# RIKEN-RCCS/EigenExa

Measured on AMD Instinct MI355X. Metric: eigen_sx full-solve throughput (reference flop model: 4/3 N^3 + D&C GEMM + 2 nvec N^2), higher is better.
Workload: dtype f64; 1 GPU; N=8192 random symmetric fp64 (counter-based R+R^T, seed 20240807), eigen_sx all eigenpairs, m_forward=64, m_backward=128; parallelism=1 GPU (1x1 grid)

## Files before the change

### eigenexa_amd/csrc/api.hip

```cpp
#include "eigx_context.h"
#include "eigx_comm.h"
#include "../../include/eigenexa_amd.h"
#include <cstring>

namespace eigx {
Context g_ctx;
}

using namespace eigx;

extern "C" {

int eigx_init(int device) {
  return eigx_init_multi(device, 0, 1, nullptr, 'C');
}

int eigx_get_device_count(void) {
  int ndev = 0;
  if (hipGetDeviceCount(&ndev) != hipSuccess) { (void)hipGetLastError(); return 0; }
  return ndev;
}

int eigx_get_rccl_unique_id(void* out128) {
  return comm_get_unique_id(out128);
}

static int g_next_px = 0, g_next_py = 0;
int eigx_set_grid_dims(int px, int py) {
  if (px < 0 || py < 0 || (px == 0) != (py == 0)) return EIGX_ERR_BAD_ARG;
  g_next_px = px; g_next_py = py;
  return EIGX_OK;
}

int eigx_init_multi(int device, int rank, int nranks, const void* uid, char order) {
  if (g_ctx.initialized) {
    fprintf(stderr, "[eigx] caution: eigx_init called twice; freeing the previous grid\n");
    eigx_free();
  }
  if (nranks < 1 || rank < 0 || rank >= nranks) return EIGX_ERR_BAD_ARG;
  int ndev = 0;
  if (hipGetDeviceCount(&ndev) != hipSuccess || ndev <= 0) {
    fprintf(stderr, "[eigx] no HIP device visible: this library has no CPU path\n");
    return EIGX_ERR_NO_DEVICE;
  }
  if (device < 0 || device >= ndev) return EIGX_ERR_BAD_ARG;
  EIGX_HIP_CHECK(hipSetDevice(device));
  g_ctx.device = device;
  int Px = 1;
  for (int x = 1; x * x <= nranks; ++x)
    if (nranks % x == 0) Px = x;
  int req_px = 0, req_py = 0;
  if (g_next_px > 0) {
    const int rx = g_next_px, ry = g_next_py;
    req_px = rx; req_py = ry;
    g_next_px = g_next_py = 0;
    if (rx * ry != nranks) {
      fprintf(stderr, "[eigx] illegal grid dimensions %d x %d for %d ranks\n", rx, ry, nranks);
      return EIGX_ERR_BAD_ARG;
    }
    Px = rx;
  }
  Grid g;
  g.Px = Px;
  g.Py = nranks / Px;
  g.rank = rank;
  g.nranks = nranks;
  if (order == 'R' || order == 'r') {
    g.px = rank / g.Py;
    g.py = rank % g.Py;
    g.row_major = 1;
  } else {
    g.px = rank % g.Px;
    g.py = rank / g.Px;
    g.row_major = 0;
  }
  g_ctx.grid = g;
  if (nranks > 1) {
    const int rc = comm_init(g_ctx, uid);
    if (rc != 0) {
      g_ctx.grid = Grid();
      g_next_px = req_px; g_next_py = req_py;
      return rc;
    }
  }
  EIGX_HIP_CHECK(hipStreamCreateWithFlags(&g_ctx.stream, hipStreamNonBlocking));
  EIGX_HIP_CHECK(hipStreamCreateWithFlags(&g_ctx.side_stream, hipStreamNonBlocking));
  for (int q = 0; q < Context::kAux; ++q)
    EIGX_HIP_CHECK(hipStreamCreateWithFlags(&g_ctx.aux[q], hipStreamNonBlocking));
  for (int q = 0; q <= Context::kAux; ++q)
    EIGX_HIP_CHECK(hipEventCreateWithFlags(&g_ctx.aux_ev[q], hipEventDisableTiming));
  EIGX_HIP_CHECK(hipEventCreateWithFlags(&g_ctx.bt_ev, hipEventDisableTiming));
  EIGX_HIP_CHECK(hipEventCreateWithFlags(&g_ctx.dc_ev, hipEventDisableTiming));
  {
    int prio_lo = 0, prio_hi = 0;
    EIGX_HIP_CHECK(hipDeviceGetStreamPriorityRange(&prio_lo, &prio_hi));
    EIGX_HIP_CHECK(hipStreamCreateWithPriority(&g_ctx.dc_stream, hipStreamNonBlocking, prio_hi));
  }
  EIGX_HIP_CHECK(hipEventCreateWithFlags(&g_ctx.dc_b_ev, hipEventDisableTiming));
  EIGX_HIP_CHECK(hipEventCreateWithFlags(&g_ctx.dc_z_ev, hipEventDisableTiming));
  g_ctx.bt_stream = g_ctx.side_stream;
  g_ctx.initialized = true;
  g_ctx.errinfo = 0;
  return EIGX_OK;
}

int eigx_free(void) {
  if (!g_ctx.initialized) return EIGX_OK;
  EIGX_HIP_CHECK(hipSetDevice(g_ctx.device));
  EIGX_HIP_CHECK(hipDeviceSynchronize());
  if (g_ctx.grid.nranks > 1) comm_free(g_ctx);
  g_ctx.pool.release();
  for (hipEvent_t e : g_ctx.prof_ev) EIGX_HIP_CHECK(hipEventDestroy(e));
  EIGX_HIP_CHECK(hipStreamDestroy(g_ctx.stream));
  EIGX_HIP_CHECK(hipStreamDestroy(g_ctx.side_stream));
  for (int q = 0; q < Context::kAux; ++q) EIGX_HIP_CHECK(hipStreamDestroy(g_ctx.aux[q]));
  for (int q = 0; q <= Context::kAux; ++q) EIGX_HIP_CHECK(hipEventDestroy(g_ctx.aux_ev[q]));
  EIGX_HIP_CHECK(hipEventDestroy(g_ctx.bt_ev));
  EIGX_HIP_CHECK(hipEventDestroy(g_ctx.dc_ev));
  EIGX_HIP_CHECK(hipStreamDestroy(g_ctx.dc_stream));
  g_ctx.bt_stream = nullptr;
  EIGX_HIP_CHECK(hipEventDestroy(g_ctx.dc_b_ev));
  EIGX_HIP_CHECK(hipEventDestroy(g_ctx.dc_z_ev));
  g_ctx = Context();
  return EIGX_OK;
}

int eigx_get_version(int* version, char* date32, char* vcode32) {
  if (version) *version = 10;
  if (date32) { memset(date32, 0, 32); strncpy(date32, "2026-10", 31); }
  if (vcode32) { memset(vcode32, 0, 32); strncpy(vcode32, "eigenexa_amd gfx950", 31); }
  return EIGX_OK;
}

int eigx_get_procs(int* procs, int* x_procs, int* y_procs) {
  if (!g_ctx.initialized) return EIGX_ERR_NOT_INITIALIZED;
  if (procs) *procs = g_ctx.grid.nranks;
  if (x_procs) *x_procs = g_ctx.grid.Px;
  if (y_procs) *y_procs = g_ctx.grid.Py;
  return EIGX_OK;
}

int eigx_get_id(int* id, int* x_id, int* y_id) {
  if (!g_ctx.initialized) return EIGX_ERR_NOT_INITIALIZED;
  if (id) *id = g_ctx.grid.rank + 1;
  if (x_id) *x_id = g_ctx.grid.px + 1;
  if (y_id) *y_id = g_ctx.grid.py + 1;
  return EIGX_OK;
}

int eigx_get_comm(int* x_color, int* x_key, int* y_color, int* y_key) {
  if (!g_ctx.initialized) return EIGX_ERR_NOT_INITIALIZED;
  const Grid& g = g_ctx.grid;
  if (x_color) *x_color = g.py + 1;
  if (x_key) *x_key = g.px + 1;
  if (y_color) *y_color = g.px + 1;
  if (y_key) *y_key = g.py + 1;
  return EIGX_OK;
}

double eigx_comm_seconds(void) { return g_ctx.timers[4]; }

int eigx_comm_info(char* buf, int len) {
  if (!g_ctx.initialized) return EIGX_ERR_NOT_INITIALIZED;
  return comm_info(g_ctx, buf, len);
}

int eigx_get_errinfo(int64_t* info) {
  if (info) *info = g_ctx.errinfo;
  return EIGX_OK;
}

int eigx_loop_start(int istart, int nnod, int inod) { return (istart + nnod - 1 - inod) / nnod + 1; }
int eigx_loop_end(int iend, int nnod, int inod) { return (iend + nnod - inod) / nnod; }
int eigx_translate_l2g(int ictr, int nnod, int inod) { return (ictr - 1) * nnod + inod; }
int eigx_translate_g2l(int ictr, int nnod, int inod) { (void)inod; return (ictr - 1) / nnod + 1; }
int eigx_owner_node(int ictr, int nnod, int inod) { (void)inod; return (ictr - 1) % nnod + 1; }
int eigx_owner_index(int ictr, int nnod, int inod) {
  return ((ictr - 1) % nnod + 1 == inod) ? (ictr - 1) / nnod + 1 : -1;
}

int eigx_matdims_for_grid(int n, int x_procs, int y_procs, int m_forward, int m_backward, char mode, int* nx, int* ny) {
  if (!nx || !ny || x_procs < 1 || y_procs < 1) return EIGX_ERR_BAD_ARG;
  (void)m_forward;
  if (n <= 0) { *nx = -1; *ny = -1; return EIGX_ERR_BAD_ARG; }
  const int Px = x_procs, Py = y_procs;
  const int mb = m_backward > 0 ? m_backward : 128;
  const int n1 = ceil_div(n, Px);
  const int n2 = ceil_div(n, Py);
  int lnx;
  int64_t lny;
  if (mode == 'M' || mode == 'm') {
    lnx = n1; lny = n2;
  } else if (mode == 'L' || mode == 'l') {
    lnx = ceil_div(n1, 32) * 32; lny = n2;
  } else {
    lnx = ceil_div(n1, 64) * 64 + 32;
    if (lnx < n1 + 64) lnx += 64;
    const int NB = mb > 64 ? mb : 64;
    int64_t nmz = (int64_t)ceil_div(n1, NB) * NB + 1;
    const int64_t nmz2 = (int64_t)ceil_div(ceil_div(n, NB), Px) * NB;
    if (nmz2 > nmz) nmz = nmz2;
    int64_t nmw = (int64_t)ceil_div(n2, NB) * NB + 1;
    const int64_t nmw2 = (int64_t)ceil_div(ceil_div(n, NB), Py) * NB;
    if (nmw2 > nmw) nmw = nmw2;
    nmz += NB; nmw += NB;
    const int64_t big = nmz > lnx ? nmz : lnx;
    lny = ceil_div64(big * nmw, lnx);
    if (lny < n2) lny = n2;
    lnx = hbm_ld(lnx);
  }
  {
    const int P = Px * Py;
    const int nf = ceil_div(n, P);
    const int64_t nx0 = (int64_t)nf * (P / Px), ny0 = (int64_t)nf * (P / Py);
    if (nx0 > lnx) lnx = (int)nx0;
    if (ny0 > lny) lny = ny0;
  }
  const int pmin = Px < Py ? Px : Py;
  const int64_t side = ceil_div64(ceil_div(n, pmin), 64) * 64;
  if ((side * side >= ((int64_t)1 << 31) || lny >= ((int64_t)1 << 31)) && !(getenv("EIGX_ALLOW_64BIT"))) {
    *nx = -1; *ny = -1;
    return EIGX_ERR_TOO_LARGE;
  }
  *nx = lnx;
  *ny = (int)lny;
  return EIGX_OK;
}

int eigx_get_matdims(int n, int* nx, int* ny, int m_forward, int m_backward, char mode) {
  if (!g_ctx.initialized) return EIGX_ERR_NOT_INITIALIZED;
  return eigx_matdims_for_grid(n, g_ctx.grid.Px, g_ctx.grid.Py, m_forward, m_backward, mode, nx, ny);
}

int64_t eigx_memory_internal(int n, int lda, int ldz, int m_forward, int m_backward) {
  if (!g_ctx.initialized) return -1;
  return solver_workspace_bytes(g_ctx, n, lda, ldz, m_forward, m_backward);
}

int64_t eigx_held_bytes(void) {
  if (!g_ctx.initialized) return -1;
  int64_t t = 0;
  for (const auto& kv : g_ctx.pool.bufs) t += (int64_t)kv.second.bytes;
  return t + comm_held_bytes(g_ctx);
}

int64_t eigx_held_bytes_named(const char* prefix) {
  if (!g_ctx.initialized || !prefix) return -1;
  const std::string pre(prefix);
  int64_t t = 0;
  for (const auto& kv : g_ctx.pool.bufs)
    if (kv.first.compare(0, pre.size(), pre) == 0) t += (int64_t)kv.second.bytes;
  return t;
}

int eigx_get_timers(double* out16) {
  if (!out16) return EIGX_ERR_BAD_ARG;
  for (int i = 0; i < 16; ++i) out16[i] = g_ctx.timers[i];
  return EIGX_OK;
}

int eigx_profile(int stride) {
  if (!g_ctx.initialized) return EIGX_ERR_NOT_INITIALIZED;
  g_ctx.prof_stride = stride > 0 ? stride : 0;
  g_ctx.prof_used = 0;
  g_ctx.prof_kind.clear();
  g_ctx.prof_units.clear();
  return EIGX_OK;
}

int eigx_profile_read(double* out6) {
  if (!g_ctx.initialized) return EIGX_ERR_NOT_INITIALIZED;
  if (!out6) return EIGX_ERR_BAD_ARG;
  EIGX_HIP_CHECK(hipSetDevice(g_ctx.device));
  EIGX_HIP_CHECK(hipStreamSynchronize(g_ctx.stream));
  for (int q = 0; q < 6; ++q) out6[q] = 0.0;
  for (size_t q = 0; q < g_ctx.prof_kind.size(); ++q) {
    float ms = 0.f;
    EIGX_HIP_CHECK(hipEventElapsedTime(&ms, g_ctx.prof_ev[2 * q], g_ctx.prof_ev[2 * q + 1]));
    if (g_ctx.prof_kind[q] > 1) continue;
    const int k = g_ctx.prof_kind[q] ? 3 : 0;
    out6[k + 0] += 1.0;
    out6[k + 1] += g_ctx.prof_units[q];
    out6[k + 2] += 1e-3 * ms;
  }
  return EIGX_OK;
}

int eigx_profile_read_kinds(double* out, int nkinds) {
  if (!g_ctx.initialized) return EIGX_ERR_NOT_INITIALIZED;
  if (!out || nkinds < 1) return EIGX_ERR_BAD_ARG;
  EIGX_HIP_CHECK(hipSetDevice(g_ctx.device));
  EIGX_HIP_CHECK(hipStreamSynchronize(g_ctx.stream));
  for (int q = 0; q < 3 * nkinds; ++q) out[q] = 0.0;
  for (size_t q = 0; q < g_ctx.prof_kind.size(); ++q) {
    const int k = g_ctx.prof_kind[q];
    if (k < 0 || k >= nkinds) continue;
    float ms = 0.f;
    EIGX_HIP_CHECK(hipEventElapsedTime(&ms, g_ctx.prof_ev[2 * q], g_ctx.prof_ev[2 * q + 1]));
    out[3 * k + 0] += 1.0;
    out[3 * k + 1] += g_ctx.prof_units[q];
    out[3 * k + 2] += 1e-3 * ms;
  }
  return EIGX_OK;
}

int eigx_device_synchronize(void) {
  if (!g_ctx.initialized) return EIGX_ERR_NOT_INITIALIZED;
  EIGX_HIP_CHECK(hipSetDevice(g_ctx.device));
  EIGX_HIP_CHECK(hipDeviceSynchronize());
  return EIGX_OK;
}

void* eigx_malloc_dev(int64_t bytes) {
  if (!g_ctx.initialized) return nullptr;
  void* p = nullptr;
  if (hipMalloc(&p, (size_t)bytes) != hipSuccess) return nullptr;
  return p;
}
int eigx_free_dev(void* p) {
  if (p) EIGX_HIP_CHECK(hipFree(p));
  return EIGX_OK;
}
int eigx_memcpy_h2d(void* dst, const void* src, int64_t bytes) {
  EIGX_HIP_CHECK(hipMemcpy(dst, src, (size_t)bytes, hipMemcpyHostToDevice));
  return EIGX_OK;
}
int eigx_memcpy_d2h(void* dst, const void* src, int64_t bytes) {
  EIGX_HIP_CHECK(hipMemcpy(dst, src, (size_t)bytes, hipMemcpyDeviceToHost));
  return EIGX_OK;
}

int eigx_tune(int key, int value) {
  if (key == 0) return set_gemm_variant(value);
  if (key == 1) return set_bisect_threads(value);
  if (key == 2) return set_bt_q(value);
  if (key == 3 || key == 4 || key == 5 || key == 10 || key == 11) return set_reduce_knob(key, value);
  if (key == 12) return (value >= 0 && value <= 2) ? set_reduce_knob(key, value) : -1;
  if (key == 6) return set_gemm_cstream(value);
  if (key == 7) return value > 0 ? set_reduce_knob(key, value) : -1;
  if (key == 8) return set_dc_chunk(value);
  if (key == 9) return comm_set_bounce(value);
  if (key == 15) return set_dc_pipe(value);
  if (key == 16) return set_dc_batch(value);
  if (key == 17 || key == 18 || key == 19) return set_range_knob(key, value);
  if (key == 20) return set_tri_nb(value);
  if (key == 21) return set_batch_nmax(value);
  if (key == 22) return set_hbatch_nmax(value);
  if (key == 23) return set_gbatch_nmax(value);
  if (key == 24) return set_hgbatch_nmax(value);
  return -1;
}

int eigx_dgemm_dev(char opa, char opb, int m, int n, int k, double alpha, const double* a, int lda,
                   const double* b, int ldb, double beta, double* c, int ldc, int tri_upper) {
  if (!g_ctx.initialized) return EIGX_ERR_NOT_INITIALIZED;
  EIGX_HIP_CHECK(hipStreamSynchronize(nullptr));
  dgemm_dev(g_ctx.stream, opa, opb, m, n, k, alpha, a, lda, b, ldb, beta, c, ldc, tri_upper ? 1 : 0,
            &g_ctx.grid);
  EIGX_HIP_CHECK(hipStreamSynchronize(g_ctx.stream));
  return EIGX_OK;
}

int eigx_dgemm_gather_dev(char opa, char opb, int m, int n, int k, double alpha, const double* a, int lda,
                          const double* b, int ldb, double beta, double* c, int ldc, const int* kmap_a,
                          const int* kmap_b) {
  if (!g_ctx.initialized) return EIGX_ERR_NOT_INITIALIZED;
  EIGX_HIP_CHECK(hipStreamSynchronize(nullptr));
  dgemm_dev(g_ctx.stream, opa, opb, m, n, k, alpha, a, lda, b, ldb, beta, c, ldc, 0, nullptr, kmap_a, nullptr, 1, 0,
            0, 0, 1, 0, 0, 0, 1, 0, kmap_b);
  EIGX_HIP_CHECK(hipStreamSynchronize(g_ctx.stream));
  return EIGX_OK;
}

}
```

### eigenexa_amd/csrc/eigx_common.h

```cpp
#pragma once
#include <hip/hip_runtime.h>
#include <cstdio>
#include <cstdlib>
#include <cstdint>
#include <cmath>
#include <vector>
#include <ctime>
#include <chrono>

#define EIGX_HIP_CHECK(expr)                                                        \
  do {                                                                              \
    hipError_t _e = (expr);                                                         \
    if (_e != hipSuccess) {                                                         \
      fprintf(stderr, "[eigx] HIP error %s at %s:%d: %s\n", hipGetErrorName(_e),    \
              __FILE__, __LINE__, hipGetErrorString(_e));                           \
      abort();                                                                      \
    }                                                                               \
  } while (0)

namespace eigx {

typedef double d4_t __attribute__((ext_vector_type(4)));

struct Grid {
  int Px = 1, Py = 1;
  int px = 0, py = 0;
  int rank = 0, nranks = 1;
  int row_major = 0;
};

static inline int ceil_div(int a, int b) { return (a + b - 1) / b; }

static inline int hbm_ld(int l) {
  if (l < 2048) return l;
  const int m = l % 2048;
  if (m < 512) return l + (512 - m);
  if (m > 1536) return l + (2048 - m) + 512;
  return l;
}
static inline int pad_ld(int n) {
  static const int extra = [] { const char* e = getenv("EIGX_LD_EXTRA"); return e ? atoi(e) : 0; }();
  int l = (n + 31) / 32;
  if (l * 32 >= 2048) return hbm_ld(l * 32) + extra;
  if ((l & 1) == 0) ++l;
  return l * 32 + extra;
}
static inline int64_t ceil_div64(int64_t a, int64_t b) { return (a + b - 1) / b; }

static inline int local_count(int n, int P, int p) { return n > p ? (n - p + P - 1) / P : 0; }
static inline int numroc(int n, int nb, int p, int P) {
  const int nblocks = n / nb;
  int cnt = (nblocks / P) * nb;
  const int extra = nblocks % P;
  if (p < extra) cnt += nb;
  else if (p == extra) cnt += n % nb;
  return cnt;
}

inline double now_s() {
  return std::chrono::duration<double>(std::chrono::steady_clock::now().time_since_epoch()).count();
}

struct SolveRequest {
  char mode;
  int nvec;
  bool want_vec;
};
inline char upper_case(char c) { return (c >= 'a' && c <= 'z') ? (char)(c - 'a' + 'A') : c; }
inline SolveRequest normalize_request(int n, int nvec, char mode) {
  mode = upper_case(mode);
  if (nvec == 0) mode = 'N';
  if (nvec < 0) nvec = -nvec;
  if (nvec > n) nvec = n;
  return SolveRequest{mode, nvec, mode != 'N'};
}


__global__ void fill_kernel(double* p, size_t n, double v);
__global__ void fill_vec_kernel(double* __restrict__ w, int n, double v);
__global__ void scale_vec_kernel(double* __restrict__ w, int n, double s);

void dgemm_dev(hipStream_t stream, char opA, char opB, int M, int N, int K, double alpha,
               const double* A, int lda, const double* B, int ldb, double beta, double* C, int ldc,
               int tri_mode = 0, const Grid* g = nullptr, const int* kmapA = nullptr,
               const int* cmapC = nullptr, int batch = 1, long strideA = 0, long strideB = 0, long strideC = 0,
               int batch2 = 1, long strideA2 = 0, long strideB2 = 0, long strideC2 = 0, int ownP = 1,
               int ownp = 0, const int* kmapB = nullptr, int tn_lo = 0, int tn_hi = 0x7fffffff);

struct GemmBatch {
  int M, N, K, pad;
  long offA, offB, offC;
  int offKA, offKB;
};
void dgemm_gather_batch_dev(hipStream_t stream, const GemmBatch* tab_dev, int nbatch, int maxM, int maxN,
                            const double* A, int lda, const double* B, int ldb, double* C, int ldc,
                            const int* kmapA, const int* kmapB);

inline void stage_trace(int rank, const char* what, long detail = -1) {
  static const bool on = getenv("EIGX_TRACE_STAGES") != nullptr;
  if (!on) return;
  timespec ts;
  clock_gettime(CLOCK_MONOTONIC, &ts);
  if (detail >= 0) fprintf(stderr, "[eigx stage] rank %d t=%.3f %s %ld\n", rank, ts.tv_sec % 100000 + ts.tv_nsec * 1e-9, what, detail);
  else fprintf(stderr, "[eigx stage] rank %d t=%.3f %s\n", rank, ts.tv_sec % 100000 + ts.tv_nsec * 1e-9, what);
  fflush(stderr);
}

int set_gemm_variant(int v);
int set_gemm_cstream(int v);
int set_bisect_threads(int v);
int set_bt_q(int v);
int set_reduce_knob(int key, int v);
int set_dc_chunk(int v);
int set_dc_pipe(int v);
int set_dc_batch(int v);
int set_batch_nmax(int v);
int set_hbatch_nmax(int v);
int set_gbatch_nmax(int v);
int set_hgbatch_nmax(int v);

}
```

### eigenexa_amd/csrc/gemm_f64.hip

```cpp
#include "eigx_common.h"

namespace eigx {

namespace {

constexpr int BK = 16;
constexpr int LD_KC = BK + 1;
template <int WT> struct Geo {
  static constexpr int BM = 2 * WT, BN = 2 * WT;
  static constexpr int LD_MC = BM + 16;
  static constexpr int OPER = (BK * LD_MC > BM * LD_KC) ? BK * LD_MC : BM * LD_KC;
  static constexpr int NL = BM * BK / 256;
  static constexpr int NF = WT / 16;
};

struct GemmArgs {
  int M, N, K;
  double alpha, beta;
  const double* A;
  int lda;
  const double* B;
  int ldb;
  double* C;
  int ldc;
  int tri_mode;
  int Px, px, Py, py;
  const int* kmapA;
  const int* cmapC;
  const int* kmapB;
  long sA, sB, sC;
  long sA2, sB2, sC2;
  int ownP, ownp;
  int tri_gb;
  int tn_lo, tn_hi;
  int c_stream;
  int nrg, rg_h, rg_c1;
  unsigned rg_magic;
  const GemmBatch* btab;
};
__host__ __device__ inline int tri2_c0(const GemmArgs& g, int q, int tiles_n) {
  const long grow_min = (long)q * g.rg_h * 128 * g.Px + g.px;
  const unsigned x = grow_min > g.py ? (unsigned)(grow_min - g.py + g.Py - 1) : 0u;
#ifdef __HIP_DEVICE_COMPILE__
  const unsigned lc = (g.Py == 1) ? x : __umulhi(x, g.rg_magic);
#else
  const unsigned lc = (g.Py == 1) ? x : (unsigned)(((unsigned long long)x * g.rg_magic) >> 32);
#endif
  int c = (lc > (unsigned)(g.N - 1)) ? tiles_n : (int)(lc >> 7);
  if (c < g.tn_lo) c = g.tn_lo;
  if (c > g.rg_c1) c = g.rg_c1;
  return c;
}
typedef double d2s_t __attribute__((ext_vector_type(2)));

template <int WT>
__device__ __forceinline__ void load_map(int (&kc)[Geo<WT>::NL], const int* __restrict__ kmap, int k0, int Kmax,
                                         int tid) {
  constexpr int BM = Geo<WT>::BM, NL = Geo<WT>::NL;
  const int kb = k0 + tid / BM;
#pragma unroll
  for (int p = 0; p < NL; ++p) {
    const int k = kb + (256 / BM) * p;
    kc[p] = kmap[k < Kmax ? k : 0];
  }
}

template <bool KC, int WT, bool MAP>
__device__ __forceinline__ void load_slab(double (&r)[Geo<WT>::NL], const double* __restrict__ P, int ld, int m0,
                                          int k0, int Mmax, int Kmax, int tid, const int (&kc)[Geo<WT>::NL]) {
  constexpr int BM = Geo<WT>::BM, NL = Geo<WT>::NL;
  if (!KC) {
    const int m = m0 + (tid & (BM - 1));
    const int kb = k0 + tid / BM;
    const bool mok = m < Mmax;
    if (MAP) {
#pragma unroll
      for (int p = 0; p < NL; ++p) {
        const int k = kb + (256 / BM) * p;
        r[p] = (mok && k < Kmax) ? P[(size_t)m + (size_t)kc[p] * ld] : 0.0;
      }
    } else {
#pragma unroll
      for (int p = 0; p < NL; ++p) {
        const int k = kb + (256 / BM) * p;
        r[p] = (mok && k < Kmax) ? P[(size_t)m + (size_t)k * ld] : 0.0;
      }
    }
  } else {
    const int k = k0 + (tid & 15);
    const int mb = m0 + (tid >> 4);
    const bool kok = k < Kmax;
#pragma unroll
    for (int p = 0; p < NL; ++p) {
      const int m = mb + 16 * p;
      r[p] = (kok && m < Mmax) ? P[(size_t)k + (size_t)m * ld] : 0.0;
    }
  }
}

template <bool KC, int WT>
__device__ __forceinline__ void store_slab(const double (&r)[Geo<WT>::NL], double* __restrict__ S, int tid) {
  constexpr int BM = Geo<WT>::BM, NL = Geo<WT>::NL, LD_MC = Geo<WT>::LD_MC;
  if (!KC) {
    const int m = tid & (BM - 1);
    const int kb = tid / BM;
#pragma unroll
    for (int p = 0; p < NL; ++p) S[(kb + (256 / BM) * p) * LD_MC + m] = r[p];
  } else {
    const int k = tid & 15;
    const int mb = tid >> 4;
#pragma unroll
    for (int p = 0; p < NL; ++p) S[(mb + 16 * p) * LD_KC + k] = r[p];
  }
}

template <bool KC, int WT>
__device__ __forceinline__ double frag(const double* __restrict__ S, int m, int k) {
  return KC ? S[m * LD_KC + k] : S[k * Geo<WT>::LD_MC + m];
}

template <bool A_KC, bool B_KC, int WT, bool GATHER>
__global__ __launch_bounds__(256, 2) void gemm_f64_kernel(GemmArgs g) {
  extern __shared__ __attribute__((aligned(16))) double smem[];
  constexpr int BM = Geo<WT>::BM, BN = Geo<WT>::BN, OPER_DOUBLES = Geo<WT>::OPER, NL = Geo<WT>::NL, NF = Geo<WT>::NF;
  g.A += (long)blockIdx.y * g.sA + (long)blockIdx.z * g.sA2;
  g.B += (long)blockIdx.y * g.sB + (long)blockIdx.z * g.sB2;
  g.C += (long)blockIdx.y * g.sC + (long)blockIdx.z * g.sC2;
  if (g.btab) {
    const GemmBatch b = g.btab[blockIdx.y];
    g.M = b.M; g.N = b.N; g.K = b.K;
    g.A += b.offA; g.B += b.offB; g.C += b.offC;
    if (GATHER) { g.kmapA += b.offKA; g.kmapB += b.offKB; }
    if ((int)blockIdx.x >= ((g.M + BM - 1) / BM) * ((g.N + BN - 1) / BN)) return;
  }

  const int tid = threadIdx.x;
  const int lane = tid & 63;
  const int wave = tid >> 6;
  const int wm = wave & 1, wn = wave >> 1;

  int bid = blockIdx.x;
  const int tiles_m = (g.M + BM - 1) / BM;
  const int tiles_n = (g.N + BN - 1) / BN;
  const int ntiles = tiles_m * tiles_n;
  int tm, tn;
  if (g.tri_mode == 1 && tiles_n % 8 == 0) {
    const int xcd = bid & 7, idx = bid >> 3;
    tn = 8 * (idx / tiles_m) + xcd;
    tm = idx % tiles_m;
  } else {
    if (g.tri_mode == 0 && ntiles % 8 == 0) bid = (bid & 7) * (ntiles >> 3) + (bid >> 3);
    tm = bid % tiles_m;
    tn = bid / tiles_m;
  }
  const int m0 = tm * BM, n0 = tn * BN;

  if (g.tri_mode != 0) {
    if (g.ownP > 1 && (tn % g.ownP) != g.ownp) return;
    if (tn < g.tn_lo || tn >= g.tn_hi) return;
    const long grow_min = (long)m0 * g.Px + g.px;
    const int jmax = (n0 + BN - 1 < g.N - 1) ? n0 + BN - 1 : g.N - 1;
    const long gcol_max = (long)jmax * g.Py + g.py;
    if (grow_min > gcol_max) return;
  }

  const int fm = lane & 15, fk = lane >> 4;
  d4_t acc[NF][NF];
  const bool use_c = (g.beta != 0.0) && (g.alpha != 0.0);
  if (use_c) {
    const double cscale = g.beta / g.alpha;
#pragma unroll
    for (int j = 0; j < NF; ++j)
#pragma unroll
      for (int r = 0; r < 4; ++r) {
        const int n = n0 + wn * WT + j * 16 + fk + 4 * r;
        const int nc = (g.cmapC && n < g.N) ? g.cmapC[n] : n;
        const double* cp = g.C + (size_t)nc * g.ldc;
#pragma unroll
        for (int i = 0; i < NF; ++i) {
          const int m = m0 + wm * WT + i * 16 + fm;
          acc[i][j][r] = (n < g.N && m < g.M) ? cscale * cp[m] : 0.0;
        }
      }
  } else {
#pragma unroll
    for (int j = 0; j < NF; ++j)
#pragma unroll
      for (int i = 0; i < NF; ++i) acc[i][j] = (d4_t){0.0, 0.0, 0.0, 0.0};
  }

  double ra[NL], rb[NL];
  int kca[NL], kcb[NL];
#pragma unroll
  for (int p = 0; p < NL; ++p) { kca[p] = 0; kcb[p] = 0; }
  const int nk = (g.K + BK - 1) / BK;
  if (GATHER) { load_map<WT>(kca, g.kmapA, 0, g.K, tid); load_map<WT>(kcb, g.kmapB, 0, g.K, tid); }
  load_slab<A_KC, WT, GATHER>(ra, g.A, g.lda, m0, 0, g.M, g.K, tid, kca);
  load_slab<B_KC, WT, GATHER>(rb, g.B, g.ldb, n0, 0, g.N, g.K, tid, kcb);
  if (GATHER && nk > 1) { load_map<WT>(kca, g.kmapA, BK, g.K, tid); load_map<WT>(kcb, g.kmapB, BK, g.K, tid); }
  store_slab<A_KC, WT>(ra, smem, tid);
  store_slab<B_KC, WT>(rb, smem + OPER_DOUBLES, tid);
  __syncthreads();

  for (int kt = 0; kt < nk; ++kt) {
    const int cur = kt & 1;
    if (kt + 1 < nk) {
      load_slab<A_KC, WT, GATHER>(ra, g.A, g.lda, m0, (kt + 1) * BK, g.M, g.K, tid, kca);
      load_slab<B_KC, WT, GATHER>(rb, g.B, g.ldb, n0, (kt + 1) * BK, g.N, g.K, tid, kcb);
      if (GATHER && kt + 2 < nk) {
        load_map<WT>(kca, g.kmapA, (kt + 2) * BK, g.K, tid);
        load_map<WT>(kcb, g.kmapB, (kt + 2) * BK, g.K, tid);
      }
    }
    const double* as = smem + cur * 2 * OPER_DOUBLES;
    const double* bs = as + OPER_DOUBLES;
#pragma unroll
    for (int ks = 0; ks < BK / 4; ++ks) {
      double fa[NF], fb[NF];
#pragma unroll
      for (int i = 0; i < NF; ++i) fa[i] = frag<A_KC, WT>(as, wm * WT + i * 16 + fm, ks * 4 + fk);
#pragma unroll
      for (int j = 0; j < NF; ++j) fb[j] = frag<B_KC, WT>(bs, wn * WT + j * 16 + fm, ks * 4 + fk);
#pragma unroll
      for (int j = 0; j < NF; ++j)
#pragma unroll
        for (int i = 0; i < NF; ++i)
          acc[i][j] = __builtin_amdgcn_mfma_f64_16x16x4f64(fb[j], fa[i], acc[i][j], 0, 0, 0);
    }
    if (kt + 1 < nk) {
      store_slab<A_KC, WT>(ra, smem + (cur ^ 1) * 2 * OPER_DOUBLES, tid);
      store_slab<B_KC, WT>(rb, smem + (cur ^ 1) * 2 * OPER_DOUBLES + OPER_DOUBLES, tid);
    }
    __syncthreads();
  }

  const double alpha = g.alpha, beta = g.beta;
#pragma unroll
  for (int j = 0; j < NF; ++j) {
#pragma unroll
    for (int r = 0; r < 4; ++r) {
      const int n = n0 + wn * WT + j * 16 + fk + 4 * r;
      if (n >= g.N) continue;
      const int nc = g.cmapC ? g.cmapC[n] : n;
      double* cp = g.C + (size_t)nc * g.ldc;
#pragma unroll
      for (int i = 0; i < NF; ++i) {
        const int m = m0 + wm * WT + i * 16 + fm;
        if (m < g.M) {
          double v = alpha * acc[i][j][r];
          if (alpha == 0.0 && beta != 0.0) v = beta * cp[m];
          cp[m] = v;
        }
      }
    }
  }
}


constexpr int G2_BK = 8;
constexpr int G2_STAGE = 2 * G2_BK * 128;

__device__ double g_zero_page[128];

__device__ __forceinline__ void glds16(const double* gp, double* lp) {
  const unsigned lds_off = (unsigned)(uintptr_t)(__attribute__((address_space(3))) void*)lp;
  asm volatile("s_mov_b32 m0, %1\n\ts_nop 0\n\tglobal_load_lds_dwordx4 %0, off" ::"v"(gp), "s"(lds_off) : "memory");
}

template <bool KC>
__device__ __forceinline__ void g2_issue(const double* __restrict__ P, int ld, int x0, int Xmax, int k0, int K,
                                         double* img, int wave, int lane, int col0, int col1) {
  if (!KC) {
    int x = x0 + 2 * lane;
    if (x + 1 >= Xmax) x = (Xmax - 1) & ~1;
#pragma unroll
    for (int q = 0; q < 2; ++q) {
      const int kr = 2 * wave + q;
      const int k = k0 + kr;
      const int col = q ? col1 : col0;
      const double* src = (k < K) ? P + (size_t)x + (size_t)col * ld : g_zero_page + 2 * lane;
      glds16(src, img + kr * 128);
    }
  } else {
#pragma unroll
    for (int q = 0; q < 2; ++q) {
      const int blk = 2 * wave + q;
      int x = x0 + blk * 16 + (lane >> 2);
      if (x >= Xmax) x = Xmax - 1;
      const int ch = (lane & 3) ^ ((lane >> 4) & 3);
      const int k = k0 + 2 * ch;
      const double* src = (k < K) ? P + (size_t)k + (size_t)x * ld : g_zero_page + 2 * lane;
      glds16(src, img + blk * 128);
    }
  }
}

__device__ __forceinline__ int g2_sload(const int* p, int idx) {
  int v;
  asm volatile("s_load_dword %0, %1, %2" : "=s"(v) : "s"(p), "s"(idx * 4) : "memory");
  return v;
}
template <bool MAP>
__device__ __forceinline__ void g2_cols(const int* __restrict__ kmap, int k0, int K, int wave, int& c0, int& c1) {
  const int k = k0 + 2 * wave;
  if (MAP) {
    c0 = 0; c1 = 0;
    if (k < K) c0 = g2_sload(kmap, k);
    if (k + 1 < K) c1 = g2_sload(kmap, k + 1);
  } else {
    c0 = k; c1 = k + 1;
  }
}

template <bool A_KC, bool B_KC, bool GATHER>
__global__ __launch_bounds__(256, 2) void gemm2_kernel(GemmArgs g) {
  extern __shared__ __attribute__((aligned(16))) double smem[];
  constexpr int S = 4;
  constexpr int GI = 4;
  g.A += (long)blockIdx.y * g.sA + (long)blockIdx.z * g.sA2;
  g.B += (long)blockIdx.y * g.sB + (long)blockIdx.z * g.sB2;
  g.C += (long)blockIdx.y * g.sC + (long)blockIdx.z * g.sC2;

  const int tid = threadIdx.x;
  const int lane = tid & 63;
  const int wave = __builtin_amdgcn_readfirstlane(tid >> 6);
  const int wm = wave & 1, wn = wave >> 1;

  const int tiles_m = (g.M + 127) / 128;
  const int tiles_n = (g.N + 127) / 128;
  int tm, tn;
  if (g.tri_mode == 1) {
    const int GB = g.tri_gb;
    const int xcd = blockIdx.x & 7, seq = blockIdx.x >> 3;
    const int blk = (seq / (GB * GB)) * 8 + xcd;
    const int w = seq % (GB * GB);
    int bj = (int)((sqrt(8.0 * blk + 1.0) - 1.0) * 0.5);
    while ((bj + 1) * (bj + 2) / 2 <= blk) ++bj;
    while (bj * (bj + 1) / 2 > blk) --bj;
    const int bi = blk - bj * (bj + 1) / 2;
    tm = bi * GB + (w % GB);
    tn = bj * GB + (w / GB);
    if (tm >= tiles_m || tn >= tiles_n) return;
  } else if (g.tri_mode == 2 && g.nrg > 0) {
    int o = blockIdx.x;
    {
      const int ntiles = (int)gridDim.x;
      const int q = ntiles >> 3, r = ntiles & 7, xcd = o & 7;
      o = (xcd < r ? xcd * (q + 1) : r * (q + 1) + (xcd - r) * q) + (o >> 3);
    }
    int rg = 0, st0 = 0, c0 = 0;
    for (int q = 0; q < g.nrg; ++q) {
      const int c = tri2_c0(g, q, tiles_n);
      const int rws = (tiles_m - q * g.rg_h < g.rg_h) ? tiles_m - q * g.rg_h : g.rg_h;
      const int cnt = rws * (g.rg_c1 - c);
      rg = q; c0 = c;
      if (o < st0 + cnt) break;
      st0 += cnt;
    }
    const int rem = o - st0;
    const int rows = (tiles_m - rg * g.rg_h < g.rg_h) ? tiles_m - rg * g.rg_h : g.rg_h;
    const int tc = rem / rows;
    tn = c0 + tc;
    tm = rg * g.rg_h + rem - tc * rows;
  } else {
    const int ntiles = tiles_m * tiles_n;
    int o = blockIdx.x;
    {
      const int q = ntiles >> 3, r = ntiles & 7, xcd = o & 7;
      o = (xcd < r ? xcd * (q + 1) : r * (q + 1) + (xcd - r) * q) + (o >> 3);
    }
    const int rg = o / (8 * tiles_n);
    const int rem = o - rg * 8 * tiles_n;
    const int rows = (tiles_m - rg * 8 < 8) ? tiles_m - rg * 8 : 8;
    tn = rem / rows;
    tm = rg * 8 + rem - tn * rows;
  }
  const int m0 = tm * 128, n0 = tn * 128;
  if (g.tri_mode != 0) {
    if (g.ownP > 1 && (tn % g.ownP) != g.ownp) return;
    if (tn < g.tn_lo || tn >= g.tn_hi) return;
    const long grow_min = (long)m0 * g.Px + g.px;
    const int jmax = (n0 + 127 < g.N - 1) ? n0 + 127 : g.N - 1;
    const long gcol_max = (long)jmax * g.Py + g.py;
    if (grow_min > gcol_max) return;
  }

  const int fm = lane & 15, fk = lane >> 4;
  const int nk = (g.K + G2_BK - 1) / G2_BK;

  auto ncol = [&](int j, int rho) { return B_KC ? j * 16 + rho : (j >> 1) * 32 + 2 * rho + (j & 1); };

  d4_t acc[4][4];
  const bool use_c = (g.beta != 0.0) && (g.alpha != 0.0);
  if (use_c) {
    const double cscale = g.beta / g.alpha;
#pragma unroll
    for (int j = 0; j < 4; ++j)
#pragma unroll
      for (int r = 0; r < 4; ++r) {
        const int n = n0 + wn * 64 + ncol(j, fk + 4 * r);
        const double* cp = g.C + (size_t)n * g.ldc;
        if (!A_KC) {
#pragma unroll
          for (int p = 0; p < 2; ++p) {
            const int m = m0 + wm * 64 + p * 32 + 2 * fm;
            double2 v = make_double2(0.0, 0.0);
            if (n < g.N) {
              if (m + 1 < g.M) {
                if (g.c_stream) { const d2s_t t = __builtin_nontemporal_load(reinterpret_cast<const d2s_t*>(cp + m)); v = make_double2(t.x, t.y); }
                else v = *reinterpret_cast<const double2*>(cp + m);
              } else if (m < g.M) v.x = cp[m];
            }
            acc[2 * p][j][r] = cscale * v.x;
            acc[2 * p + 1][j][r] = cscale * v.y;
          }
        } else {
#pragma unroll
          for (int i = 0; i < 4; ++i) {
            const int m = m0 + wm * 64 + i * 16 + fm;
            acc[i][j][r] = (n < g.N && m < g.M) ? cscale * cp[m] : 0.0;
          }
        }
      }
  } else {
#pragma unroll
    for (int j = 0; j < 4; ++j)
#pragma unroll
      for (int i = 0; i < 4; ++i) acc[i][j] = (d4_t){0.0, 0.0, 0.0, 0.0};
  }

  int ca0, ca1, cb0, cb1;
#pragma unroll
  for (int s = 0; s < S - 1; ++s) {
    double* st = smem + s * G2_STAGE;
    g2_cols<GATHER && !A_KC>(g.kmapA, s * G2_BK, g.K, wave, ca0, ca1);
    g2_cols<GATHER && !B_KC>(g.kmapB, s * G2_BK, g.K, wave, cb0, cb1);
    if (GATHER) asm volatile("s_waitcnt lgkmcnt(0)" : "+s"(ca0), "+s"(ca1), "+s"(cb0), "+s"(cb1)::"memory");
    g2_issue<A_KC>(g.A, g.lda, m0, g.M, s * G2_BK, g.K, st, wave, lane, ca0, ca1);
    g2_issue<B_KC>(g.B, g.ldb, n0, g.N, s * G2_BK, g.K, st + G2_BK * 128, wave, lane, cb0, cb1);
  }
  g2_cols<GATHER && !A_KC>(g.kmapA, (S - 1) * G2_BK, g.K, wave, ca0, ca1);
  g2_cols<GATHER && !B_KC>(g.kmapB, (S - 1) * G2_BK, g.K, wave, cb0, cb1);

  for (int kt = 0; kt < nk; ++kt) {
    if (GATHER)
      asm volatile("s_waitcnt vmcnt(%4) lgkmcnt(0)\n\ts_barrier"
                   : "+s"(ca0), "+s"(ca1), "+s"(cb0), "+s"(cb1) : "n"((S - 2) * GI) : "memory");
    else
      asm volatile("s_waitcnt vmcnt(%0)\n\ts_barrier" ::"n"((S - 2) * GI) : "memory");
    {
      const int ks = kt + S - 1;
      double* st = smem + (ks % S) * G2_STAGE;
      g2_issue<A_KC>(g.A, g.lda, m0, g.M, ks * G2_BK, g.K, st, wave, lane, ca0, ca1);
      g2_issue<B_KC>(g.B, g.ldb, n0, g.N, ks * G2_BK, g.K, st + G2_BK * 128, wave, lane, cb0, cb1);
      g2_cols<GATHER && !A_KC>(g.kmapA, (ks + 1) * G2_BK, g.K, wave, ca0, ca1);
      g2_cols<GATHER && !B_KC>(g.kmapB, (ks + 1) * G2_BK, g.K, wave, cb0, cb1);
    }
    const double* as = smem + (kt % S) * G2_STAGE;
    const double* bs = as + G2_BK * 128;
#pragma unroll
    for (int ks = 0; ks < G2_BK / 4; ++ks) {
      const int k = ks * 4 + fk;
      double fa[4], fb[4];
      if (!A_KC) {
#pragma unroll
        for (int p = 0; p < 2; ++p) {
          const double2 v = *reinterpret_cast<const double2*>(as + k * 128 + wm * 64 + p * 32 + 2 * fm);
          fa[2 * p] = v.x; fa[2 * p + 1] = v.y;
        }
      } else {
#pragma unroll
        for (int i = 0; i < 4; ++i) {
          const int m = wm * 64 + i * 16 + fm;
          fa[i] = as[m * 8 + (((k >> 1) ^ ((m >> 2) & 3)) << 1) + (k & 1)];
        }
      }
      if (!B_KC) {
#pragma unroll
        for (int p = 0; p < 2; ++p) {
          const double2 v = *reinterpret_cast<const double2*>(bs + k * 128 + wn * 64 + p * 32 + 2 * fm);
          fb[2 * p] = v.x; fb[2 * p + 1] = v.y;
        }
      } else {
#pragma unroll
        for (int j = 0; j < 4; ++j) {
          const int n = wn * 64 + j * 16 + fm;
          fb[j] = bs[n * 8 + (((k >> 1) ^ ((n >> 2) & 3)) << 1) + (k & 1)];
        }
      }
#pragma unroll
      for (int j = 0; j < 4; ++j)
#pragma unroll
        for (int i = 0; i < 4; ++i)
          acc[i][j] = __builtin_amdgcn_mfma_f64_16x16x4f64(fb[j], fa[i], acc[i][j], 0, 0, 0);
    }
  }
  asm volatile("s_waitcnt vmcnt(0)" ::: "memory");

  const double alpha = g.alpha;
#pragma unroll
  for (int j = 0; j < 4; ++j) {
#pragma unroll
    for (int r = 0; r < 4; ++r) {
      const int n = n0 + wn * 64 + ncol(j, fk + 4 * r);
      if (n >= g.N) continue;
      double* cp = g.C + (size_t)n * g.ldc;
      if (!A_KC) {
#pragma unroll
        for (int p = 0; p < 2; ++p) {
          const int m = m0 + wm * 64 + p * 32 + 2 * fm;
          const double2 v = make_double2(alpha * acc[2 * p][j][r], alpha * acc[2 * p + 1][j][r]);
          if (m + 1 < g.M) {
            if (g.c_stream) { d2s_t t; t.x = v.x; t.y = v.y; __builtin_nontemporal_store(t, reinterpret_cast<d2s_t*>(cp + m)); }
            else *reinterpret_cast<double2*>(cp + m) = v;
          } else if (m < g.M) cp[m] = v.x;
        }
      } else {
#pragma unroll
        for (int i = 0; i < 4; ++i) {
          const int m = m0 + wm * 64 + i * 16 + fm;
          if (m < g.M) cp[m] = alpha * acc[i][j][r];
        }
      }
    }
  }
}

int g_gemm_cstream = 0;
int g_gemm_variant = 2;

static bool gemm2_ok(const GemmArgs& g, bool a_kc, bool b_kc, int batch, int batch2) {
  if (g_gemm_variant < 2) return false;
  if (g.M < 2 || g.N < 2 || g.K < 1 || g.alpha == 0.0 || g.cmapC) return false;
  if ((g.lda | g.ldb | g.ldc) & 1) return false;
  if (((uintptr_t)g.A | (uintptr_t)g.B | (uintptr_t)g.C) & 15) return false;
  if (batch > 1 && ((g.sA | g.sB | g.sC) & 1)) return false;
  if (batch2 > 1 && ((g.sA2 | g.sB2 | g.sC2) & 1)) return false;
  if ((a_kc || b_kc) && (g.K & 1)) return false;
  if (a_kc && g.lda < g.K) return false;
  if (b_kc && g.ldb < g.K) return false;
  return true;
}

}

int set_gemm_variant(int v) { const int old = g_gemm_variant; g_gemm_variant = v; return old; }
int set_gemm_cstream(int v) { const int old = g_gemm_cstream; g_gemm_cstream = v; return old; }

void dgemm_dev(hipStream_t stream, char opA, char opB, int M, int N, int K, double alpha, const double* A,
               int lda, const double* B, int ldb, double beta, double* C, int ldc, int tri_mode,
               const Grid* grid, const int* kmapA, const int* cmapC, int batch, long strideA, long strideB,
               long strideC, int batch2, long strideA2, long strideB2, long strideC2, int ownP, int ownp,
               const int* kmapB, int tn_lo, int tn_hi) {
  if (M <= 0 || N <= 0 || batch <= 0 || batch2 <= 0) return;
  GemmArgs g;
  g.M = M; g.N = N; g.K = K; g.alpha = alpha; g.beta = beta;
  g.A = A; g.lda = lda; g.B = B; g.ldb = ldb; g.C = C; g.ldc = ldc;
  g.tri_mode = tri_mode;
  g.kmapA = (opA == 'N' || opA == 'n') ? kmapA : nullptr;
  g.cmapC = cmapC;
  g.kmapB = (opB == 'T' || opB == 't') ? kmapB : nullptr;
  g.sA = strideA; g.sB = strideB; g.sC = strideC;
  g.sA2 = strideA2; g.sB2 = strideB2; g.sC2 = strideC2;
  g.ownP = ownP; g.ownp = ownp; g.tri_gb = 1;
  g.tn_lo = tn_lo; g.tn_hi = tn_hi;
  g.nrg = 0; g.rg_h = 8; g.rg_c1 = 0; g.rg_magic = 0; g.btab = nullptr;
  g.c_stream = (tri_mode != 0 && g_gemm_cstream) ? 1 : 0;
  g.Px = grid ? grid->Px : 1; g.px = grid ? grid->px : 0;
  g.Py = grid ? grid->Py : 1; g.py = grid ? grid->py : 0;
  const bool a_kc = (opA == 'T' || opA == 't');
  const bool b_kc = (opB == 'N' || opB == 'n');
  const bool gather = g.kmapA || g.kmapB;
  if ((!gather || (g.kmapA && g.kmapB && !a_kc && !b_kc)) && gemm2_ok(g, a_kc, b_kc, batch, batch2)) {
    const long t128 = (long)ceil_div(M, 128) * ceil_div(N, 128) * batch * batch2;
    if (tri_mode != 0 || t128 >= 192 || g_gemm_variant == 3) {
      int gx2 = ceil_div(M, 128) * ceil_div(N, 128);
      if (tri_mode == 1) {
        const int t = ceil_div(N > M ? N : M, 128);
        g.tri_gb = (t >= 96) ? 8 : (t >= 24 ? 4 : (t >= 8 ? 2 : 1));
        const int nb = ceil_div(t, g.tri_gb);
        const int nblk = nb * (nb + 1) / 2;
        gx2 = 8 * ceil_div(nblk, 8) * g.tri_gb * g.tri_gb;
      }
      if (tri_mode == 2 && batch == 1 && batch2 == 1 && ownP == 1) {
        const int tiles_m = ceil_div(M, 128), tiles_n = ceil_div(N, 128);
        g.rg_h = (tiles_m <= 256) ? 8 : ceil_div(tiles_m, 32);
        g.nrg = ceil_div(tiles_m, g.rg_h);
        g.rg_c1 = tiles_n < tn_hi ? tiles_n : tn_hi;
        g.rg_magic = (unsigned)(((1ull << 32) / (unsigned long long)g.Py) + 1ull);
        int total = 0;
        for (int q = 0; q < g.nrg; ++q) {
          const int rows = (tiles_m - q * g.rg_h < g.rg_h) ? tiles_m - q * g.rg_h : g.rg_h;
          total += rows * (g.rg_c1 - tri2_c0(g, q, tiles_n));
        }
        if (total == 0) return;
        gx2 = total;
      }
      dim3 grd2(gx2, batch, batch2), blk2(256);
      const size_t shmem2 = (size_t)4 * G2_STAGE * sizeof(double);
#define EIGX_LAUNCH2(AK, BK_, GA_)                                                                 \
  do {                                                                                             \
    static bool attr_set2 = false;                                                                 \
    if (!attr_set2) {                                                                              \
      EIGX_HIP_CHECK(hipFuncSetAttribute((const void*)gemm2_kernel<AK, BK_, GA_>,                  \
                                         hipFuncAttributeMaxDynamicSharedMemorySize, (int)shmem2)); \
      attr_set2 = true;                                                                            \
    }                                                                                              \
    hipLaunchKernelGGL((gemm2_kernel<AK, BK_, GA_>), grd2, blk2, shmem2, stream, g);               \
  } while (0)
      if (gather) EIGX_LAUNCH2(false, false, true);
      else if (a_kc && b_kc) EIGX_LAUNCH2(true, true, false);
      else if (a_kc) EIGX_LAUNCH2(true, false, false);
      else if (b_kc) EIGX_LAUNCH2(false, true, false);
      else EIGX_LAUNCH2(false, false, false);
#undef EIGX_LAUNCH2
      EIGX_HIP_CHECK(hipGetLastError());
      return;
    }
  }
  const long tiles128 = (long)ceil_div(M, 128) * ceil_div(N, 128) * batch * batch2;
  const bool small = (tri_mode == 0) && tiles128 < 192;
  const int bm = small ? 64 : 128;
  const int tiles = ceil_div(M, bm) * ceil_div(N, bm);
  dim3 grd(tiles, batch, batch2), blk(256);
#define EIGX_LAUNCH(AK, BK_, WT_, GA_)                                                             \
  do {                                                                                             \
    const size_t shmem = (size_t)4 * Geo<WT_>::OPER * sizeof(double);                              \
    static bool attr_set = false;                                                                  \
    if (!attr_set) {                                                                               \
      EIGX_HIP_CHECK(hipFuncSetAttribute((const void*)gemm_f64_kernel<AK, BK_, WT_, GA_>,          \
                                         hipFuncAttributeMaxDynamicSharedMemorySize, (int)shmem)); \
      attr_set = true;                                                                             \
    }                                                                                              \
    hipLaunchKernelGGL((gemm_f64_kernel<AK, BK_, WT_, GA_>), grd, blk, shmem, stream, g);          \
  } while (0)
#define EIGX_LAUNCH_T(AK, BK_) do { if (small) EIGX_LAUNCH(AK, BK_, 32, false); else EIGX_LAUNCH(AK, BK_, 64, false); } while (0)
  if (g.kmapA || g.kmapB) {
    if (a_kc || b_kc || !g.kmapA || !g.kmapB) {
      fprintf(stderr, "[eigx] dgemm gather needs opA='N', opB='T' and both maps\n");
      abort();
    }
    if (small) EIGX_LAUNCH(false, false, 32, true); else EIGX_LAUNCH(false, false, 64, true);
  } else if (a_kc && b_kc) EIGX_LAUNCH_T(true, true);
  else if (a_kc && !b_kc) EIGX_LAUNCH_T(true, false);
  else if (!a_kc && b_kc) EIGX_LAUNCH_T(false, true);
  else EIGX_LAUNCH_T(false, false);
#undef EIGX_LAUNCH_T
#undef EIGX_LAUNCH
  EIGX_HIP_CHECK(hipGetLastError());
}

void dgemm_gather_batch_dev(hipStream_t stream, const GemmBatch* tab_dev, int nbatch, int maxM, int maxN,
                            const double* A, int lda, const double* B, int ldb, double* C, int ldc,
                            const int* kmapA, const int* kmapB) {
  if (nbatch <= 0 || maxM <= 0 || maxN <= 0) return;
  GemmArgs g;
  g.M = maxM; g.N = maxN; g.K = 0; g.alpha = 1.0; g.beta = 0.0;
  g.A = A; g.lda = lda; g.B = B; g.ldb = ldb; g.C = C; g.ldc = ldc;
  g.tri_mode = 0; g.kmapA = kmapA; g.cmapC = nullptr; g.kmapB = kmapB;
  g.sA = g.sB = g.sC = 0; g.sA2 = g.sB2 = g.sC2 = 0;
  g.ownP = 1; g.ownp = 0; g.tri_gb = 1; g.tn_lo = 0; g.tn_hi = 0x7fffffff;
  g.nrg = 0; g.rg_h = 8; g.rg_c1 = 0; g.rg_magic = 0; g.c_stream = 0;
  g.Px = 1; g.px = 0; g.Py = 1; g.py = 0;
  g.btab = tab_dev;
  constexpr int WT = 32;
  const int tiles = ceil_div(maxM, Geo<WT>::BM) * ceil_div(maxN, Geo<WT>::BN);
  const size_t shmem = (size_t)4 * Geo<WT>::OPER * sizeof(double);
  static bool attr_set = false;
  if (!attr_set) {
    EIGX_HIP_CHECK(hipFuncSetAttribute((const void*)gemm_f64_kernel<false, false, WT, true>,
                                       hipFuncAttributeMaxDynamicSharedMemorySize, (int)shmem));
    attr_set = true;
  }
  hipLaunchKernelGGL((gemm_f64_kernel<false, false, WT, true>), dim3(tiles, nbatch, 1), dim3(256), shmem, stream, g);
  EIGX_HIP_CHECK(hipGetLastError());
}

}
```

Before: 19280 GFLOP/s.

## Defer C loading to the pipeline tail in gemm2 for short-K triangular updates

Adds a LATE_C variant of gemm2_kernel that skips preloading C into the accumulators. Instead it issues the C tile loads during the last three pipelined k-slabs and combines alpha*AB + beta*C at store time, interleaving C loads for later column groups with stores of earlier ones. The aim is to hide C-read latency behind MFMA work for short-K rank-k triangular updates (tri_mode 1, K <= 256 by default, plain N/T operands), such as the tridiagonalization trailing updates. In exchange it costs extra registers for the staged C values, which could lower occupancy, and it assumes there are at least three k-slabs.

```diff
diff --git a/eigenexa_amd/csrc/api.hip b/eigenexa_amd/csrc/api.hip
--- a/eigenexa_amd/csrc/api.hip
+++ b/eigenexa_amd/csrc/api.hip
@@ -348,6 +348,7 @@
   if (key == 22) return set_hbatch_nmax(value);
   if (key == 23) return set_gbatch_nmax(value);
   if (key == 24) return set_hgbatch_nmax(value);
+  if (key == 25) return set_gemm_latec_kmax(value);
   return -1;
 }
 
diff --git a/eigenexa_amd/csrc/eigx_common.h b/eigenexa_amd/csrc/eigx_common.h
--- a/eigenexa_amd/csrc/eigx_common.h
+++ b/eigenexa_amd/csrc/eigx_common.h
@@ -108,6 +108,7 @@
 
 int set_gemm_variant(int v);
 int set_gemm_cstream(int v);
+int set_gemm_latec_kmax(int v);
 int set_bisect_threads(int v);
 int set_bt_q(int v);
 int set_reduce_knob(int key, int v);
diff --git a/eigenexa_amd/csrc/gemm_f64.hip b/eigenexa_amd/csrc/gemm_f64.hip
--- a/eigenexa_amd/csrc/gemm_f64.hip
+++ b/eigenexa_amd/csrc/gemm_f64.hip
@@ -312,11 +312,13 @@
   }
 }
 
-template <bool A_KC, bool B_KC, bool GATHER>
+template <bool A_KC, bool B_KC, bool GATHER, bool LATE_C = false>
 __global__ __launch_bounds__(256, 2) void gemm2_kernel(GemmArgs g) {
+  static_assert(!LATE_C || (!A_KC && !B_KC && !GATHER), "late C: plain 'N','T' operands only");
   extern __shared__ __attribute__((aligned(16))) double smem[];
   constexpr int S = 4;
   constexpr int GI = 4;
+  constexpr int CI = 8;
   g.A += (long)blockIdx.y * g.sA + (long)blockIdx.z * g.sA2;
   g.B += (long)blockIdx.y * g.sB + (long)blockIdx.z * g.sB2;
   g.C += (long)blockIdx.y * g.sC + (long)blockIdx.z * g.sC2;
@@ -391,7 +393,7 @@
   auto ncol = [&](int j, int rho) { return B_KC ? j * 16 + rho : (j >> 1) * 32 + 2 * rho + (j & 1); };
 
   d4_t acc[4][4];
-  const bool use_c = (g.beta != 0.0) && (g.alpha != 0.0);
+  const bool use_c = !LATE_C && (g.beta != 0.0) && (g.alpha != 0.0);
   if (use_c) {
     const double cscale = g.beta / g.alpha;
 #pragma unroll
@@ -442,7 +444,8 @@
   g2_cols<GATHER && !A_KC>(g.kmapA, (S - 1) * G2_BK, g.K, wave, ca0, ca1);
   g2_cols<GATHER && !B_KC>(g.kmapB, (S - 1) * G2_BK, g.K, wave, cb0, cb1);
 
-  for (int kt = 0; kt < nk; ++kt) {
+  const int nk_ring = LATE_C ? ((nk > S - 1 ? nk : S - 1) - (S - 1)) : nk;
+  for (int kt = 0; kt < nk_ring; ++kt) {
     if (GATHER)
       asm volatile("s_waitcnt vmcnt(%4) lgkmcnt(0)\n\ts_barrier"
                    : "+s"(ca0), "+s"(ca1), "+s"(cb0), "+s"(cb1) : "n"((S - 2) * GI) : "memory");
@@ -495,6 +498,88 @@
           acc[i][j] = __builtin_amdgcn_mfma_f64_16x16x4f64(fb[j], fa[i], acc[i][j], 0, 0, 0);
     }
   }
+
+  if constexpr (LATE_C) {
+    double2 cv[4][4][2];
+    const double* const zero16 = g_zero_page + 2 * lane;
+    typedef const __attribute__((address_space(1))) d2s_t* c16_t;
+    auto c_load = [&](int j) {
+#pragma unroll
+      for (int r = 0; r < 4; ++r) {
+        const int n = n0 + wn * 64 + ncol(j, fk + 4 * r);
+        const double* col = g.C + (size_t)n * g.ldc;
+#pragma unroll
+        for (int p = 0; p < 2; ++p) {
+          const int m = m0 + wm * 64 + p * 32 + 2 * fm;
+          c16_t src = (c16_t)((n < g.N && m + 1 < g.M) ? col + m : zero16);
+          asm volatile("" : "+v"(src));
+          const d2s_t t = *src;
+          cv[j][r][p] = make_double2(t.x, t.y);
+        }
+      }
+    };
+    auto mul_slab = [&](int kt) {
+      const double* as = smem + (kt % S) * G2_STAGE;
+      const double* bs = as + G2_BK * 128;
+#pragma unroll
+      for (int ks = 0; ks < G2_BK / 4; ++ks) {
+        const int k = ks * 4 + fk;
+        double fa[4], fb[4];
+#pragma unroll
+        for (int p = 0; p < 2; ++p) {
+          const double2 va = *reinterpret_cast<const double2*>(as + k * 128 + wm * 64 + p * 32 + 2 * fm);
+          const double2 vb = *reinterpret_cast<const double2*>(bs + k * 128 + wn * 64 + p * 32 + 2 * fm);
+          fa[2 * p] = va.x; fa[2 * p + 1] = va.y;
+          fb[2 * p] = vb.x; fb[2 * p + 1] = vb.y;
+        }
+#pragma unroll
+        for (int j = 0; j < 4; ++j)
+#pragma unroll
+          for (int i = 0; i < 4; ++i)
+            acc[i][j] = __builtin_amdgcn_mfma_f64_16x16x4f64(fb[j], fa[i], acc[i][j], 0, 0, 0);
+      }
+    };
+    const int kt0 = nk_ring;
+    asm volatile("s_waitcnt vmcnt(%0)\n\ts_barrier" ::"n"((S - 2) * GI) : "memory");
+    c_load(0); c_load(1);
+    mul_slab(kt0);
+    asm volatile("s_waitcnt vmcnt(%0)\n\ts_barrier" ::"n"((S - 3) * GI + 2 * CI) : "memory");
+    mul_slab(kt0 + 1);
+    asm volatile("s_waitcnt vmcnt(%0)\n\ts_barrier" ::"n"(2 * CI) : "memory");
+    mul_slab(kt0 + 2);
+
+    const double alpha = g.alpha, beta = g.beta;
+    auto combine = [&](int j) {
+#pragma unroll
+      for (int r = 0; r < 4; ++r)
+#pragma unroll
+        for (int p = 0; p < 2; ++p) {
+          acc[2 * p][j][r] = alpha * acc[2 * p][j][r] + beta * cv[j][r][p].x;
+          acc[2 * p + 1][j][r] = alpha * acc[2 * p + 1][j][r] + beta * cv[j][r][p].y;
+        }
+    };
+    auto store = [&](int j) {
+#pragma unroll
+      for (int r = 0; r < 4; ++r) {
+        const int n = n0 + wn * 64 + ncol(j, fk + 4 * r);
+        if (n >= g.N) continue;
+        double* cp = g.C + (size_t)n * g.ldc;
+#pragma unroll
+        for (int p = 0; p < 2; ++p) {
+          const int m = m0 + wm * 64 + p * 32 + 2 * fm;
+          if (m + 1 < g.M) *reinterpret_cast<double2*>(cp + m) = make_double2(acc[2 * p][j][r], acc[2 * p + 1][j][r]);
+          else if (m < g.M) cp[m] = acc[2 * p][j][r] + beta * cp[m];
+        }
+      }
+    };
+#pragma unroll
+    for (int j = 0; j < 4; ++j) {
+      combine(j);
+      if (j + 2 < 4) c_load(j + 2);
+      store(j);
+    }
+    return;
+  }
   asm volatile("s_waitcnt vmcnt(0)" ::: "memory");
 
   const double alpha = g.alpha;
@@ -528,6 +613,7 @@
 
 int g_gemm_cstream = 0;
 int g_gemm_variant = 2;
+int g_gemm_latec_kmax = 256;
 
 static bool gemm2_ok(const GemmArgs& g, bool a_kc, bool b_kc, int batch, int batch2) {
   if (g_gemm_variant < 2) return false;
@@ -546,6 +632,10 @@
 
 int set_gemm_variant(int v) { const int old = g_gemm_variant; g_gemm_variant = v; return old; }
 int set_gemm_cstream(int v) { const int old = g_gemm_cstream; g_gemm_cstream = v; return old; }
+int set_gemm_latec_kmax(int v) {
+  if (v < 0 || v >= 512) return -1;
+  const int old = g_gemm_latec_kmax; g_gemm_latec_kmax = v; return old;
+}
 
 void dgemm_dev(hipStream_t stream, char opA, char opB, int M, int N, int K, double alpha, const double* A,
                int lda, const double* B, int ldb, double beta, double* C, int ldc, int tri_mode,
@@ -598,21 +688,23 @@
       }
       dim3 grd2(gx2, batch, batch2), blk2(256);
       const size_t shmem2 = (size_t)4 * G2_STAGE * sizeof(double);
-#define EIGX_LAUNCH2(AK, BK_, GA_)                                                                 \
+#define EIGX_LAUNCH2(AK, BK_, GA_, LC_)                                                            \
   do {                                                                                             \
     static bool attr_set2 = false;                                                                 \
     if (!attr_set2) {                                                                              \
-      EIGX_HIP_CHECK(hipFuncSetAttribute((const void*)gemm2_kernel<AK, BK_, GA_>,                  \
+      EIGX_HIP_CHECK(hipFuncSetAttribute((const void*)gemm2_kernel<AK, BK_, GA_, LC_>,             \
                                          hipFuncAttributeMaxDynamicSharedMemorySize, (int)shmem2)); \
       attr_set2 = true;                                                                            \
     }                                                                                              \
-    hipLaunchKernelGGL((gemm2_kernel<AK, BK_, GA_>), grd2, blk2, shmem2, stream, g);               \
+    hipLaunchKernelGGL((gemm2_kernel<AK, BK_, GA_, LC_>), grd2, blk2, shmem2, stream, g);          \
   } while (0)
-      if (gather) EIGX_LAUNCH2(false, false, true);
-      else if (a_kc && b_kc) EIGX_LAUNCH2(true, true, false);
-      else if (a_kc) EIGX_LAUNCH2(true, false, false);
-      else if (b_kc) EIGX_LAUNCH2(false, true, false);
-      else EIGX_LAUNCH2(false, false, false);
+      const bool late_c = tri_mode == 1 && beta != 0.0 && K <= g_gemm_latec_kmax && !g.c_stream;
+      if (gather) EIGX_LAUNCH2(false, false, true, false);
+      else if (a_kc && b_kc) EIGX_LAUNCH2(true, true, false, false);
+      else if (a_kc) EIGX_LAUNCH2(true, false, false, false);
+      else if (b_kc) EIGX_LAUNCH2(false, true, false, false);
+      else if (late_c) EIGX_LAUNCH2(false, false, false, true);
+      else EIGX_LAUNCH2(false, false, false, false);
 #undef EIGX_LAUNCH2
       EIGX_HIP_CHECK(hipGetLastError());
       return;
```

Result: faster. 19470 GFLOP/s, median of 6 (+1.0%).
